# qingyundou/WaveRNN

Measured on AMD Instinct MI355X. Metric: audio samples/sec/GPU (22.05 kHz MoL, rnn_dims=512) + real-time factor at batch=1, higher is better.
Workload: dtype f32

## Files before the change

wavernn_amd/csrc/capi_loops.cpp:

```cpp
#include "host_ctx.h"

using namespace wrnn;
using namespace wrnn::host;

namespace {

struct DbgBuf {
    unsigned *p = nullptr;
    DbgBuf() = default;
    DbgBuf(const DbgBuf &) = delete;
    DbgBuf &operator=(const DbgBuf &) = delete;
    ~DbgBuf() {
        if (p) (void)hipFree(p);
    }
    unsigned *release() {
        unsigned *q = p;
        p = nullptr;
        return q;
    }
};

int dump_stamps(wrnn_t *h, DbgBuf &dbg, size_t n, const int (&hdr)[3], hipStream_t st) {
    std::vector<unsigned> host(n);
    HIP_TRY(h, hipStreamSynchronize(st));
// ... 190 lines not shown
            g1.B = group_rows(Bl, 1);
            g1.b0 = b0 + Bg;
        }
        HIP_TRY(h, launch_dm(a, grouped ? &g1 : nullptr, dm_lds_bytes(*h, Bg, TB), st));
        b0 += Bl;
    }
    return WRNN_OK;
}

int generate_split(wrnn_t *h, const float *cond, int B, int L, const float *noise, uint64_t seed,
                   int64_t row_offset, float *out, hipStream_t st) {
    const wrnn_config &c = h->cfg;
    const int R = c.rnn_dims, A = c.aux_dims, G = h->sGg + h->sGf, N = G * kSplitTerms;
    if (int rc = blas_on(h, st)) return rc;
    const double budget = terms_budget_floats();
    const int Lc_max = (int)std::max(1.0, std::min((double)L, budget / (double)(N + h->KX) - 1.0));
    const char *rep_env = std::getenv("WRNN_REPLICAS");
    const int reps = std::max(1, std::min(32, rep_env ? std::atoi(rep_env) : 4));
    const long long vec_max = std::max<long long>({(long long)kTermsPerUnit * R, (long long)R, (long long)c.fc_dims,
                                                   (long long)(R / kSplitUnits) * kYLine,
                                                   (long long)h->sGf * kSplitLogitLine});
    const long long rep_stride = (((vec_max + kOverRead) * 8 + 65535) / 65536) * 65536 / 8;
    const size_t need_xg = (size_t)kSplitHops * reps * rep_stride;
    HIP_TRY(h, ensure(h->d_xg, h->xg_cap, need_xg));
    if (grow(h, h->d_X, h->X_cap, (size_t)(Lc_max + 1) * h->KX) || grow(h, h->d_T, h->T_cap, (size_t)(Lc_max + 1) * N) ||
        grow(h, h->d_state, h->state_cap, (size_t)G * split_state_w(R)))
        return WRNN_EHIP;
    const char *dbg_env = std::getenv("WRNN_DEBUG_STAMPS");
    const int dbg_steps = dbg_env ? std::min(L, std::atoi(dbg_env)) : 0;
    DbgBuf dbg;
    if (dbg_steps > 0) {
        HIP_TRY(h, hipMalloc(&dbg.p, (size_t)G * dbg_steps * kStamps * 4));
        HIP_TRY(h, hipMemsetAsync(dbg.p, 0, (size_t)G * dbg_steps * kStamps * 4, st));
    }
    const float one = 1.0f, zero = 0.0f;
    for (int b0 = 0; b0 < B; ++b0) {
        HIP_TRY(h, hipMemsetAsync(h->d_xg, 0, need_xg * 8, st));
        for (int t0 = 0; t0 < L; t0 += Lc_max) {
            const int Lc = std::min(Lc_max, L - t0);
            const int rows = std::min(Lc + 1, L - t0);
            HIP_TRY(h, launch_ci_gemm(cond, h->CD, B, b0, 1, t0, rows, h->d_IW, 1 + c.feat_dims + A, h->d_Ib, R,
                                      c.feat_dims + A, h->d_X, h->KX, st));
            HIP_TRY(h, launch_pack_terms_input(cond, h->CD, B, b0, 1, t0, rows, c.feat_dims, A, R, h->KX, h->d_X, st));
            if (rocblas_sgemm(h->blas, rocblas_operation_transpose, rocblas_operation_none, N, rows, h->KX, &one,
                              h->d_sWt, h->KX, h->d_X, h->KX, &zero, h->d_T, N) != rocblas_status_success)
                return fail(h, WRNN_EHIP, "rocblas_sgemm (conditioning terms) failed");
            SplitArgs a{};
            a.gslab = h->d_sgslab;
            a.fslab = h->d_sfslab;
            a.terms = h->d_T;
            a.noise = noise;
            a.out = out;
            a.state = h->d_state;
            a.xg = h->d_xg;
            a.ctl = h->d_ctl;
            a.seed = seed;
            a.row0 = row_offset + b0;
            a.timeout_ticks = h->timeout_ticks;
            a.rep_stride = rep_stride;
            a.L = L;
            a.t0 = t0;
            a.Lc = Lc;
            a.Bt = B;
            a.b0 = b0;
            a.Gg = h->sGg;
            a.Gf = h->sGf;
            a.reps = reps;
            a.gs = h->sgs;
            a.fs = h->sfs;
            a.dbg = (b0 == 0 && t0 == 0) ? dbg.p : nullptr;
            a.dbg_steps = std::min(dbg_steps, Lc);
            HIP_TRY(h, launch_split(a, split_lds_bytes(*h), st));
        }
    }
    if (dbg.p) return dump_stamps(h, dbg, (size_t)G * dbg_steps * kStamps, {G, dbg_steps, kStamps}, st);
    return WRNN_OK;
}

template <typename Args, typename Slab>
int generate_xcd_rows(wrnn_t *h, const float *cond, const FrameSrc *fs, int B, int L, const float *noise,
                      uint64_t seed, int64_t row_offset, float *out, hipStream_t st, int n_terms, int state_w,
                      const Slab &slab, hipError_t (*launch)(const Args &, hipStream_t)) {
    const int N = kXcdWgs * n_terms;
    if (int rc = blas_on(h, st)) return rc;
    if (fs) {
        const float one = 1.0f, zero = 0.0f;
        const int rc = frame_terms(h, *fs, N, h->KXc, 0, st, [&](const float *X, int m, float *C) -> int {
            if (rocblas_sgemm(h->blas, rocblas_operation_transpose, rocblas_operation_none, N, m, h->KXc, &one,
                              h->d_xWt, h->KXc, X, h->KXc, &zero, C, N) != rocblas_status_success)
                return fail(h, WRNN_EHIP, "rocblas_sgemm (frame terms) failed");
            return WRNN_OK;
        });
        if (rc) return rc;
    }
    const double budget = terms_budget_floats();
    const size_t xg_words = (size_t)kXcds * kXXcdStride;
    if (!h->d_members) HIP_TRY(h, hipMalloc(&h->d_members, kXcds * sizeof(int)));
    if (!h->d_xgx) HIP_TRY(h, hipMalloc(&h->d_xgx, xg_words * 8));
    const char *dbg_env = std::getenv("WRNN_DEBUG_STAMPS");
    const int dbg_steps = dbg_env ? std::min(L, std::atoi(dbg_env)) : 0;
    DbgBuf dbg;
    int dbg_G = 0;
    const float one = 1.0f, zero = 0.0f;
    for (int b0 = 0; b0 < B; b0 += kXcds) {
        const int nb = std::min(kXcds, B - b0);
        const int Lc_max = (int)std::max(1.0, std::min((double)L, budget / ((double)nb * (N + h->KXc)) - 1.0));
        if (grow(h, h->d_X, h->X_cap, (size_t)(Lc_max + 1) * nb * h->KXc) ||
            grow(h, h->d_T, h->T_cap, (size_t)(Lc_max + 1) * nb * N) ||
            grow(h, h->d_xstate, h->xstate_cap, (size_t)nb * kXcdWgs * state_w))
            return WRNN_EHIP;
        if (dbg_steps > 0 && !dbg.p) {
            dbg_G = nb * kXcdWgs;
            HIP_TRY(h, hipMalloc(&dbg.p, (size_t)dbg_G * dbg_steps * kStamps * 4));
            HIP_TRY(h, hipMemsetAsync(dbg.p, 0, (size_t)dbg_G * dbg_steps * kStamps * 4, st));
        }
        HIP_TRY(h, hipMemsetAsync(h->d_xgx, 0, (size_t)nb * kXXcdStride * 8, st));
        for (int t0 = 0; t0 < L; t0 += Lc_max) {
            const int Lc = std::min(Lc_max, L - t0);
            const int rows = std::min(Lc + 1, L - t0);
            if (fs) {
                HIP_TRY(h, launch_terms_interp(h->d_FT, h->d_AT, fs->coef, h->d_T, N, fs->U, fs->NF, fs->NF + fs->nJ - 1,
                                               fs->hop, fs->nJ, fs->nf, fs->stride, fs->rb + b0, nb, t0, rows, st));
            } else {
                HIP_TRY(h, launch_pack_cond_input(cond, h->CD, B, b0, nb, t0, rows, h->KXc, h->d_X, st));
                if (rocblas_sgemm(h->blas, rocblas_operation_transpose, rocblas_operation_none, N, rows * nb, h->KXc,
                                  &one, h->d_xWt, h->KXc, h->d_X, h->KXc, &zero, h->d_T, N) != rocblas_status_success)
                    return fail(h, WRNN_EHIP, "rocblas_sgemm (conditioning terms) failed");
            }
            HIP_TRY(h, hipMemsetAsync(h->d_members, 0, kXcds * sizeof(int), st));
            Args a{};
            a.slab = h->d_xslab;
            a.terms = h->d_T;
            a.noise = noise;
            a.out = out;
            a.state = h->d_xstate;
            a.xg = h->d_xgx;
            a.members = h->d_members;
            a.ctl = h->d_ctl;
            a.seed = seed;
            a.row0 = row_offset + b0;
            a.timeout_ticks = h->timeout_ticks;
            a.L = L;
            a.t0 = t0;
            a.Lc = Lc;
            a.Bt = B;
            a.b0 = b0;
            a.nb = nb;
            a.s = slab;
            a.dbg = (b0 == 0 && t0 == 0) ? dbg.p : nullptr;
            a.dbg_steps = std::min(dbg_steps, Lc);
            HIP_TRY(h, launch(a, st));
        }
    }
    if (dbg.p) return dump_stamps(h, dbg, (size_t)dbg_G * dbg_steps * kStamps, {dbg_G, dbg_steps, kStamps}, st);
    return WRNN_OK;
}

int generate_xcd(wrnn_t *h, const float *cond, const FrameSrc *fs, int B, int L, const float *noise, uint64_t seed,
                 int64_t row_offset, float *out, hipStream_t st) {
    return generate_xcd_rows<XcdArgs>(h, cond, fs, B, L, noise, seed, row_offset, out, st, kXTerms, kXStateW, h->xs,
                                      launch_xcd);
}

int generate_xcds(wrnn_t *h, const float *cond, const FrameSrc *fs, int B, int L, const float *noise, uint64_t seed,
                  int64_t row_offset, float *out, hipStream_t st) {
    return generate_xcd_rows<XcdsArgs>(h, cond, fs, B, L, noise, seed, row_offset, out, st, kSTerms, kSStateW, h->xss,
                                       launch_xcds);
}

int generate_xcdm(wrnn_t *h, const float *cond, const FrameSrc *fs, int B, int L, const float *noise, uint64_t seed,
                  int64_t row_offset, float *out, int32_t *labels, hipStream_t st) {
    const int N = kXcdWgs * kMRing;
    const bool raw = h->cfg.mode == WRNN_MODE_RAW;
    const int NK = raw ? kMRawNC : 11;
    if (int rc = blas_on(h, st)) return rc;
    const double budget = terms_budget_floats();
    const size_t xg_words = (size_t)kXcds * kMXcdStride;
    if (!h->d_members) HIP_TRY(h, hipMalloc(&h->d_members, kXcds * sizeof(int)));
    if (!h->d_xmxg) HIP_TRY(h, hipMalloc(&h->d_xmxg, xg_words * 8));
    if (!h->d_xmstate) HIP_TRY(h, hipMalloc(&h->d_xmstate, (size_t)kXcds * kXcdWgs * kMStateW * sizeof(float)));
    const int rows_max = kXcds * 4 * h->xcdm_nq;
    const float one = 1.0f, zero = 0.0f;
    XcdmGemm gemms[3];
    xcdm_terms_gemms(*h, gemms);
    auto terms_gemm = [&](const float *X, int m, float *C) -> int {
        for (const XcdmGemm &g : gemms) {
            const rocblas_status rs =
                rocblas_sgemm(h->blas, rocblas_operation_transpose, rocblas_operation_none, g.rows, m, g.k, &one,
                              h->d_xmWt + (size_t)g.row0 * h->KXc + g.col0, h->KXc, X + g.col0, h->KXc, &zero,
                              C + g.row0, N);
            if (rs != rocblas_status_success) return fail(h, WRNN_EHIP, "rocblas_sgemm (conditioning terms) failed");
        }
        return WRNN_OK;
    };
    if (fs) {
        if (int rc = frame_terms(h, *fs, N, h->KXc, h->cfg.feat_dims + h->cfg.aux_dims, st, terms_gemm)) return rc;
    }
    const char *dbg_env = std::getenv("WRNN_DEBUG_STAMPS");
    const int dbg_steps = (!raw && dbg_env && std::atoi(dbg_env) > 0 && L >= kMDbgSkip + kMDbgSteps) ? kMDbgSteps : 0;
    const size_t dbg_n = (size_t)kXcds * kXcdWgs * kMWaves * dbg_steps * kMStamps;
    DbgBuf dbg;
    if (dbg_steps > 0) {
        HIP_TRY(h, hipMalloc(&dbg.p, dbg_n * 4));
        HIP_TRY(h, hipMemsetAsync(dbg.p, 0, dbg_n * 4, st));
    }
    for (int b0 = 0; b0 < B; b0 += rows_max) {
        const int nb = std::min(rows_max, B - b0);
        const int nq = (((nb + kXcds - 1) / kXcds) + 3) / 4;
        const int Lc_max = (int)std::max(1.0, std::min((double)L, budget / ((double)nb * (N + h->KXc + (noise ? 0 : NK)))));
        if (grow(h, h->d_X, h->X_cap, (size_t)Lc_max * nb * h->KXc) || grow(h, h->d_T, h->T_cap, (size_t)Lc_max * nb * N) ||
            (!noise && grow(h, h->d_xmnoise, h->xmnoise_cap, (size_t)Lc_max * nb * NK)))
// ... 488 lines not shown
```

wavernn_amd/csrc/fatchord_xcd.h:

```cpp
#pragma once
#include <hip/hip_runtime_api.h>
#include <stdint.h>

namespace wrnn {

constexpr int kXcds = 8;
constexpr int kXcdWgs = 32;
constexpr int kXWaves = 8;
constexpr int kXThreads = 64 * kXWaves;
constexpr int kXUnits = 16;
constexpr int kXFcRows = 16;
constexpr int kXWaveFc1 = 1, kXWaveFc2 = 3;
constexpr int kXH2RegRows = 30;
constexpr int kXH2LdsRows = 18;
static_assert(kXH2RegRows == 2 * (4 * 3 + 3 * 1), "W_hh2 VGPR passes: 3 on each fc wave, 1 on waves 5..7");
static_assert(kXH2RegRows + kXH2LdsRows == 48, "every W_hh2 row of the workgroup has one holder");
constexpr int kXRing = 4;
constexpr int kXNoise = 16;

enum XTerm { XT_P1 = 0, XT_P2 = 48, XT_CI = 96, XT_V1 = 112, XT_V2 = 128, kXTerms = 160 };

enum XHop { XH_Y = 0, XH_F1 = 1, XH_F2 = 2, XH_H2 = 3, XH_S0 = 4, XH_S1 = 5, kXHops = 6 };
constexpr int kXF2Line = 32;
constexpr long long kXHopStride = 4096;
constexpr long long kXXcdStride = kXHops * kXHopStride + 512;

struct XcdSlab {
    int wih2;
    int w1;
    int w2;
    int whh2;
    int whh1;
    int w3;
    int q1a;
    int cst;
    int total;
};

enum XCst { XC_Q2 = 0, XC_BIH1 = 48, XC_BHH1 = 96, XC_BIH2 = 144, XC_BHH2 = 192, XC_WI0 = 240, XC_B3 = 256, kXCst = 288 };

constexpr int kXStateW = 512 + 2048 + 48 + 16 + 16;

struct XcdArgs {
    const float *slab;
    const float *terms;
    const float *noise;
    float *out;
    float *state;
    unsigned long long *xg;
    int *members;
    int *ctl;
    unsigned long long seed;
    long long row0;
    long long timeout_ticks;
    int L, t0, Lc, Bt, b0, nb;
    XcdSlab s;
    unsigned *dbg;
    int dbg_steps;
    int windowed, nz_hor, out_ld, out_t0;
};

struct XcdRow {
    const float *terms;
    const float *noise;
    float *out;
    float *state;
    unsigned long long *xg;
    unsigned long long seed;
    long long row;
    long long terms_ld;
    int noise_ld;
    int out_t0;
    int t0, Lc, L, nz_hor;
};

struct XcdGroupArgs {
    XcdArgs a;
    XcdRow row[kXcds];
};

struct XcdPiece {
    XcdRow r;
    const float *ft;
    const float *at;
    int frames, nt;
    int blk0, pad_;
};

struct XcdListArgs {
    XcdArgs a;
    const XcdPiece *pieces;
    int first[kXcds + 1];
};

struct XcdLds {
    int whh1, whh2, h1, h2, sg, w3, f2x, ring, nz, gh2, cst, xs, misc, total;
};

__host__ __device__ constexpr XcdLds xcd_lds_layout() {
    XcdLds l{};
    int o = 0;
    l.h1 = o;    o += 512;
    l.h2 = o;    o += 512;
    l.sg = o;    o += 4 * 512;
    l.w3 = o;    o += kXFcRows * 32;
    l.f2x = o;   o += 64;
    l.ring = o;  o += kXRing * kXTerms;
    l.nz = o;    o += kXRing * kXNoise;
    l.gh2 = o;   o += 48;
    l.cst = o;   o += kXCst;
    l.xs = o;    o += 4;
    l.misc = o;  o += 8;
    l.whh1 = o;  o += 48 * 512;
    l.whh2 = o;  o += kXH2LdsRows * 512;
    l.total = o;
    return l;
}
static_assert(xcd_lds_layout().total * 4 <= 160 * 1024, "the XCD kernel's LDS image fits a CU's 160 KB");

hipError_t launch_xcd(const XcdArgs &a, hipStream_t st);
hipError_t launch_xcd_group(const XcdGroupArgs &g, hipStream_t st);
hipError_t launch_xcd_list(const XcdListArgs &g, hipStream_t st);
hipError_t prepare_xcd_kernel(int max_lds_bytes);
hipError_t xcd_occupancy(int *blocks_per_cu);

}
```

wavernn_amd/csrc/fatchord_xcd.hip:

```cpp
#include <hip/hip_runtime.h>
#include <stdint.h>

#include <type_traits>

#include "fatchord_loop.h"
#include "fatchord_xcd.h"
#include "wrnn_device.h"
#include "xcd_device.h"

namespace wrnn {

#ifndef WRNN_XCD_SKIP_SG
#define WRNN_XCD_SKIP_SG 0
#endif
#ifndef WRNN_XCD_SKIP_H2
#define WRNN_XCD_SKIP_H2 0
#endif
#ifndef WRNN_XCD_SKIP_RECUR
#define WRNN_XCD_SKIP_RECUR 0
#endif
#ifndef WRNN_XCD_PRIO
#define WRNN_XCD_PRIO 0
#endif

#ifndef WRNN_XCD_SQ3_WAVE
#define WRNN_XCD_SQ3_WAVE 4
#endif
#ifndef WRNN_XCD_STAMP_W13
#define WRNN_XCD_STAMP_W13 5
#endif
#define XSTAMPW(kk, w)                                                                                        \
    do {                                                                                                      \
        if (kDbg && a.dbg && wave == (w) && lane == 0 && t - t0 < a.dbg_steps &&                            \
            (!WRNN_XCD_BAR_STAMPS || ((kk) != 3 && ((kk) < 9 || (kk) > 14))))                                 \
            a.dbg[((size_t)mem * a.dbg_steps + (t - t0)) * kStamps + (kk)] = (unsigned)__builtin_amdgcn_s_memrealtime(); \
    } while (0)
#define XSTAMP(kk) XSTAMPW(kk, 0)
#define XSTAMP_BAR()                                                                                          \
    do {                                                                                                      \
        if (WRNN_XCD_BAR_STAMPS && kDbg && a.dbg && wave > 0 && lane == 0 && t - t0 < a.dbg_steps)          \
            a.dbg[((size_t)mem * a.dbg_steps + (t - t0)) * kStamps + (wave == 7 ? 3 : 8 + wave)] =          \
                (unsigned)__builtin_amdgcn_s_memrealtime();                                                   \
    } while (0)

#define XCD_PIECE_BEGIN()                                                                                     \
    do {                                                                                                      \
        {                                                                                                     \
            for (int t = t0; t < t0 + 3; ++t) {                                                               \
                if (t <= t_terms)                                                                             \
                    for (int i = tid; i < kXTerms; i += kXThreads) RING(t)[i] = TERMS(t)[i];                  \
                if (wave == 1 && lane < 11 && t < nz_hor) NZ(t)[lane] = noise_term(t);                        \
            }                                                                                                 \
        }                                                                                                     \
        resume = t0 > 0;                                                                                      \
        if constexpr (kGrp) st = rw.state + (size_t)c * kXStateW;                                             \
        else st = a.state + ((size_t)k * kXcdWgs + c) * kXStateW;                                             \
        h1v = resume ? st[tid] : 0.0f;                                                                        \
        h2own = resume ? st[512 + 2048 + 48 + ui] : 0.0f;                                                     \
        asm volatile("" : "+v"(h1v), "+v"(h2own));                                                            \
        if (resume) {                                                                                         \
            for (int i = tid; i < 4 * R; i += kXThreads) sg[i] = st[512 + i];                                 \
            if (tid < 48) gh2s[tid] = st[512 + 2048 + tid];                                                   \
            if (tid == 0) xs[(t0 + 1) & 1] = st[512 + 2048 + 48 + 16];                                        \
        } else {                                                                                              \
            if (tid < 48) gh2s[tid] = 0.0f;                                                                   \
            if (tid == 0) xs[1] = 0.0f;                                                                       \
        }                                                                                                     \
        __syncthreads();                                                                                      \
        if (!resume) {                                                                                        \
            if (gh1w) {                                                                                       \
                const float z5[5] = {0.0f, 0.0f, 0.0f, 0.0f, 0.0f};                                           \
                publish_terms(0, z5);                                                                         \
            }                                                                                                 \
            if (wave == 1 || wave == 2 || wave == 5 || wave == WRNN_XCD_SQ3_WAVE) {                           \
                asm volatile("s_waitcnt vmcnt(0)" ::: "memory");                                              \
                gather_terms(0);                                                                              \
            }                                                                                                 \
        }                                                                                                     \
        __syncthreads();                                                                                      \
        if (*abort_flag) return;                                                                              \
        x = xs[(t0 + 1) & 1];                                                                                 \
        s4 = lds4(sg + 4 * tid);                                                                              \
    } while (0)

#define XCD_PIECE_END()                                                                                       \
    do {                                                                                                      \
        __syncthreads();                                                                                      \
        st[tid] = h1v;                                                                                        \
        for (int i = tid; i < 4 * R; i += kXThreads) st[512 + i] = sg[i];                                     \
        if (tid < 48) st[512 + 2048 + tid] = gh2s[tid];                                                       \
        if (g2w && (li & ~2) == 0) st[512 + 2048 + 48 + ui] = h2own;                                          \
        if (tid == 0) st[512 + 2048 + 48 + 16] = xs[(t_end - 1) & 1];                                         \
    } while (0)

__device__ __forceinline__ const XcdArgs &launch_args(const XcdArgs &ka) { return ka; }
__device__ __forceinline__ const XcdArgs &launch_args(const XcdGroupArgs &ka) { return ka.a; }
__device__ __forceinline__ const XcdArgs &launch_args(const XcdListArgs &ka) { return ka.a; }

template <bool kDbg, bool kWin, bool kGrp = false, bool kLst = false>
__global__ __launch_bounds__(kXThreads, 2) void fatchord_xcd_kernel(
    std::conditional_t<kLst, XcdListArgs, std::conditional_t<kGrp, XcdGroupArgs, XcdArgs>> ka) {
    static_assert(!kGrp || (kWin && !kDbg), "grouped launches are windowed and carry no stamps");
    static_assert(!kLst || kGrp, "a list launch is a grouped one whose rows come from the piece queue");
    const XcdArgs &a = launch_args(ka);
    extern __shared__ __attribute__((aligned(16))) float smem[];
    constexpr int R = 512, TW = kXcdWgs * kXTerms;
    const XcdLds ll = xcd_lds_layout();
    const int tid = threadIdx.x, lane = tid & 63, li = lane & 31, eng = lane >> 5;
    const int wave = WRNN_XCD_UNIFORM_WAVE ? __builtin_amdgcn_readfirstlane(tid >> 6) : tid >> 6;
    float *whh1 = smem + ll.whh1, *whh2l = smem + ll.whh2, *f2x = smem + ll.f2x, *h1s = smem + ll.h1, *h2s = smem + ll.h2, *sg = smem + ll.sg, *w3s = smem + ll.w3;
    float *ring = smem + ll.ring, *nzr = smem + ll.nz, *gh2s = smem + ll.gh2, *cst = smem + ll.cst, *xs = smem + ll.xs;
    int *misc = reinterpret_cast<int *>(smem + ll.misc);
    int *abort_flag = misc, *h2ready = misc + 2, *ypub = misc + 3, *ygot = misc + 4, *f1got = misc + 5;

    if (tid == 0) {
        const int k = (int)xcc_id();
        int c = kXcdWgs;
        if constexpr (kLst) {
            const bool in = k < a.nb && ka.first[k + 1] > ka.first[k];
            if (in) c = atomicAdd(&a.members[k], 1);
            misc[1] = (in && c < kXcdWgs) ? k * kXcdWgs + c : -1;
        } else if constexpr (kGrp) {
            const bool in = k < a.nb && ka.row[k].Lc > 0;
            if (in) c = atomicAdd(&a.members[k], 1);
            misc[1] = (in && c < kXcdWgs) ? k * kXcdWgs + c : -1;
        } else {
            if (k < a.nb) c = atomicAdd(&a.members[k], 1);
            misc[1] = (k < a.nb && c < kXcdWgs) ? k * kXcdWgs + c : -1;
        }
        misc[0] = 0;
        for (int i = 2; i < 8; ++i) misc[i] = 0;
    }
    if (tid < 64) f2x[tid] = 0.0f;
    __syncthreads();
// ... 11 lines not shown
        t0 = rw.t0;
        Lc = rw.Lc;
        L = rw.L;
    } else if constexpr (kGrp) {
        rw = ka.row[k];
        t0 = rw.t0;
        Lc = rw.Lc;
        L = rw.L;
    } else {
        t0 = a.t0;
        Lc = a.Lc;
        L = a.L;
    }
    int t_end = t0 + Lc;
    int t_terms = min(t_end, L - 1);
    int nz_hor;
    if constexpr (kGrp) nz_hor = rw.nz_hor;
    else nz_hor = kWin ? a.nz_hor : L;
    unsigned long long *xg;
    if constexpr (kGrp) xg = rw.xg;
    else xg = a.xg + (size_t)k * kXXcdStride;
    auto XG = [&](int hop) { return xg + (size_t)hop * kXHopStride; };
    __amdgpu_buffer_rsrc_t xgr = __builtin_amdgcn_make_buffer_rsrc(xg, 0, 0x7fffffff, 0x00020000);
    auto XGI = [&](int hop) { return hop * (int)kXHopStride; };
    auto RING = [&](int t) { return ring + (t & (kXRing - 1)) * kXTerms; };
    auto NZ = [&](int t) { return nzr + (t & (kXRing - 1)) * kXNoise; };
    auto TERMS = [&](int t) {
        if constexpr (kGrp) return rw.terms + (size_t)(t - t0) * (size_t)rw.terms_ld + (size_t)c * kXTerms;
        else return a.terms + ((size_t)(t - t0) * a.nb + k) * TW + (size_t)c * kXTerms;
    };
    const float *S = a.slab + (size_t)c * a.s.total;
    unsigned long long prow, seed;
    if constexpr (kGrp) {
        prow = (unsigned long long)rw.row;
        seed = rw.seed;
    } else {
        prow = (unsigned long long)(a.row0 + k);
        seed = a.seed;
    }

    f4v W[28];
    auto ldrow = [&](const float *row, int m) { return *reinterpret_cast<const f4v *>(row + 4 * (li + 32 * m)); };
    const bool fcw = wave >= kXWaveFc1 && wave < kXWaveFc2 + 2;
    const bool g2w = !fcw;
    const int g2 = g2w && wave != 0 ? wave - 4 : 0;
    if (fcw) {
        const int hf = (wave - kXWaveFc1) & 1;
        const float *Wf = S + (wave < kXWaveFc2 ? a.s.w1 : a.s.w2) + hf * 8 * R;
#pragma unroll
        for (int p = 0; p < 4; ++p)
#pragma unroll
            for (int kk = 0; kk < 4; ++kk) {
                const f2v ra = *reinterpret_cast<const f2v *>(Wf + 2 * p * R + 2 * (lane + 64 * kk));
                const f2v rb = *reinterpret_cast<const f2v *>(Wf + (2 * p + 1) * R + 2 * (lane + 64 * kk));
                W[4 * p + kk] = f4v{ra.x, rb.x, ra.y, rb.y};
            }
#pragma unroll
        for (int p = 0; p < 3; ++p)
#pragma unroll
            for (int m = 0; m < 4; ++m) W[16 + 4 * p + m] = ldrow(S + a.s.whh2 + (2 * (3 * (wave - 1) + p) + eng) * R, m);
    } else {
        auto g2row = [&](int j, int q) { return S + a.s.wih2 + ((2 * g2 + j) * 6 + 2 * q + eng) * R; };
#pragma unroll
        for (int p = 0; p < 3; ++p) {
            const float *ra = g2row(p == 1 ? 1 : 0, p == 2 ? 2 : 0), *rb = g2row(p == 0 ? 0 : 1, p == 2 ? 2 : 1);
#pragma unroll
            for (int m = 0; m < 4; ++m) {
                const f4v wa = ldrow(ra, m), wb = ldrow(rb, m);
                W[8 * p + 2 * m] = f4v{wa.x, wb.x, wa.y, wb.y};
                W[8 * p + 2 * m + 1] = f4v{wa.z, wb.z, wa.w, wb.w};
            }
        }
#pragma unroll
        for (int m = 0; m < 4; ++m)
            W[24 + m] = wave != 0 ? ldrow(S + a.s.whh2 + (2 * (7 + wave) + eng) * R, m) : f4v{0.0f, 0.0f, 0.0f, 0.0f};
    }
    auto W4 = [&](int i) -> const f4v(&)[4] { return *reinterpret_cast<const f4v(*)[4]>(&W[i]); };
    auto W4x8 = [&](int i) -> const f4v(&)[8] { return *reinterpret_cast<const f4v(*)[8]>(&W[i]); };
    auto W4x16 = [&]() -> const f4v(&)[16] { return *reinterpret_cast<const f4v(*)[16]>(&W[0]); };
    const float q1r = S[a.s.q1a + tid], q1z = S[a.s.q1a + R + tid], q1n = S[a.s.q1a + 2 * R + tid];
    const int ui = 4 * g2 + (li & 2) + eng, gq = li & 1;
    const bool gh1w = wave == 0 || wave == 3 || wave == 4 || wave == 5 || wave == 7;
    const int gh0 = wave == 0 ? 0 : wave == 7 ? 40 : 10 * (wave - 2);
    auto noise_term = [&](int t) -> float {
        float uu;
        if constexpr (kGrp) {
            if (rw.noise) uu = rw.noise[(size_t)t * (size_t)rw.noise_ld + lane];
            else uu = philox_noise(seed, prow, (uint32_t)t, (uint32_t)lane, 1);
        } else {
            if (a.noise) uu = a.noise[((size_t)t * a.Bt + b) * 11 + lane];
            else uu = philox_noise(seed, prow, (uint32_t)t, (uint32_t)lane, 1);
        }
        return mol_noise_term(uu, lane);
    };
    auto publish_term = [&](int t, int rr, float gh) {
        const int u = rr / 3, q = rr - 3 * u;
        const float p1 = RING(t)[XT_P1 + rr], bh = cst[XC_BHH1 + rr], bi = cst[XC_BIH1 + rr];
        const int g = XGI(XH_S0 + (t & 1)) + (c * kXUnits + u) * 4;
        const uint32_t tag = (uint32_t)t + 1u;
        if (q < 2) {
            xpub_b(xgr, g + q, tag, (gh + bh) + (p1 + bi));
        } else {
            xpub_b(xgr, g + 3, tag, gh + bh);
            xpub_b(xgr, g + 2, tag, p1 + bi);
        }
    };
    auto publish_terms = [&](int t, const float (&gh)[5]) {
        const int rr = gh0 + 2 * li + eng;
        if (li < 5 && rr < 48) {
            const float v = li == 0 ? gh[0] : li == 1 ? gh[1] : li == 2 ? gh[2] : li == 3 ? gh[3] : gh[4];
            publish_term(t, rr, v);
        }
    };
    auto gh1_dots = [&](float (&gh)[5]) {
        f4v hx[4];
        e32x(h1s, li, hx);
#pragma unroll
        for (int p = 0; p < 5; ++p) {
            f4v w4[4];
            e32x(whh1 + min(gh0 + 2 * p + eng, 47) * R, li, w4);
            gh[p] = e32dot(w4, hx);
        }
    };
    auto set_flag = [&](int *f, uint32_t tag) {
        if (lane == 0) __hip_atomic_store(f, (int)tag, __ATOMIC_RELAXED, __HIP_MEMORY_SCOPE_WORKGROUP);
    };
    auto wait_flag = [&](int *f, uint32_t tag) {
        while (__hip_atomic_load(f, __ATOMIC_RELAXED, __HIP_MEMORY_SCOPE_WORKGROUP) != (int)tag)
            __builtin_amdgcn_s_sleep(1);
        asm volatile("" ::: "memory");
    };
    auto gh2_store = [&](int rb, int np, const float (&gh)[5]) {
        const int rr = rb + 2 * li + eng;
        if (li < np) gh2s[rr] = li == 0 ? gh[0] : li == 1 ? gh[1] : li == 2 ? gh[2] : li == 3 ? gh[3] : gh[4];
    };
    auto gh2_lds = [&](int p0, int np, const f4v (&hx)[4]) {
        float gh[5] = {0.0f, 0.0f, 0.0f, 0.0f, 0.0f};
#pragma unroll
        for (int p = 0; p < 2; ++p)
            if (p < np) {
                f4v w4[4];
                e32x(whh2l + (2 * (p0 + p) + eng - kXH2RegRows) * R, li, w4);
                gh[p] = e32dot(w4, hx);
            }
        gh2_store(2 * p0, np, gh);
    };
    auto gather_terms = [&](int t) {
        const int qq = wave == 1 ? 0 : wave == 2 ? 1 : wave == 5 ? 2 : 3;
        xgather16<4>(XG(XH_S0 + (t & 1)) + qq * 512, (uint32_t)t + 1u, a.ctl, a.timeout_ticks, t, XH_S0 + (t & 1),
                     abort_flag, lane, [&](int i, float v0, float v1) {
                         *reinterpret_cast<f2v *>(sg + qq * 512 + i) = f2v{v0, v1};
                     });
    };

    auto pub4 = [&](int hop, float v, uint32_t tagv) {
        const auto s = __builtin_amdgcn_permlane32_swap(__float_as_uint(v), __float_as_uint(v), false, false);
        if ((lane & ~2) == 0)
            __builtin_amdgcn_raw_buffer_store_b128(u4v{__float_as_uint(v), tagv, s[1], tagv}, xgr,
                                                   (XGI(hop) + c * kXUnits + 4 * g2 + lane) * 8, 0, 0);
    };
    {
        const f4v *src = reinterpret_cast<const f4v *>(S + a.s.whh1);
        f4v *dst = reinterpret_cast<f4v *>(whh1);
        for (int i = tid; i < 48 * R / 4; i += kXThreads) dst[i] = src[i];
        src = reinterpret_cast<const f4v *>(S + a.s.whh2 + kXH2RegRows * R);
        dst = reinterpret_cast<f4v *>(whh2l);
        for (int i = tid; i < kXH2LdsRows * R / 4; i += kXThreads) dst[i] = src[i];
        for (int i = tid; i < kXFcRows * 32; i += kXThreads) w3s[i] = S[a.s.w3 + i];
        for (int i = tid; i < kXCst; i += kXThreads) cst[i] = S[a.s.cst + i];
    }
    bool resume;
    float *st;
    float h1v, h2own;
    float x;
    f4v s4;
    XCD_PIECE_BEGIN();

    if (WRNN_XCD_PRIO && wave == 0) __builtin_amdgcn_s_setprio(WRNN_XCD_PRIO);
    for (int t = t0; t < t_end; ++t) {
        const uint32_t tag = (uint32_t)t + 1u;
        const bool more = t + 1 < L;
        const float *tr = RING(t);
        XSTAMP(0);
        if (kDbg && a.dbg && wave == 0 && lane == 0 && t - t0 < a.dbg_steps)
            a.dbg[((size_t)mem * a.dbg_steps + (t - t0)) * kStamps + 15] = (unsigned)__builtin_amdgcn_s_memtime();
        float q2v[2], p2v[2], bi2[2], ghv[2];
#pragma unroll
        for (int q = 0; q < 2; ++q) {
            const int gi = ui * 3 + (q == 0 ? gq : 2);
            q2v[q] = cst[XC_Q2 + gi];
            p2v[q] = tr[XT_P2 + gi];
            bi2[q] = cst[XC_BIH2 + gi];
            ghv[q] = gh2s[gi] + cst[XC_BHH2 + gi];
        }
        const float wi0v = cst[XC_WI0 + ui], civ = tr[XT_CI + ui];
        {
            const float r = sigmoid_(fmaf(x, q1r, s4.x));
            const float z = sigmoid_(fmaf(x, q1z, s4.y));
            const float n = tanh_(fmaf(x, q1n, s4.z) + s4.w * r);
            h1v = (h1v - n) * z + n;
            h1s[tid] = h1v;
        }
        float p2q[2];
#pragma unroll
        for (int q = 0; q < 2; ++q) p2q[q] = fmaf(x, q2v[q], p2v[q]) + bi2[q];
        const float xi = fmaf(wi0v, x, civ);
        bar();
        XSTAMP(1);
        if (g2w) {
            f4v hx[4];
            e32x(h1s, li, hx);
            float yb = xi + h1s[c * kXUnits + ui];
            uint32_t tagv = tag;
            asm volatile("" : "+v"(yb), "+v"(tagv));
            const f2v ga = e32part2(W4x8(0), hx), gb = e32part2(W4x8(8), hx);
            const float g_s = e32rs4(ga.x, ga.y, gb.x, gb.y, lane);
            const float s = sigmoid_(ghv[0] + (g_s + p2q[0]));
            const f2v gn = e32part2(W4x8(16), hx);
            const float g_n = e32rs2(gn.x, gn.y, lane);
            const float z = WRNN_DPP(s, 0xF5);
            const float n = tanh_((g_n + p2q[1]) + ghv[1] * s);
            const float hn = (h2own - n) * z + n;
            h2own = hn;
            pub4(XH_Y, yb + hn, tagv);
            if (wave == 0) set_flag(ypub, tag);
        }
        XSTAMP(2);
        auto pub_h2 = [&]() { pub4(XH_H2, h2own, tag); };
        const int jq = lane & 1, rho = jq + 2 * (lane >> 4);
        if (wave == 0) {
            if (more && !WRNN_XCD_SKIP_RECUR) {
                float gh[5];
                gh1_dots(gh);
                wait_flag(ygot, tag);
                publish_terms(t + 1, gh);
                pub_h2();
            }
            const int jp = lane & 15, pg = lane >> 4;
            const float ua = NZ(t)[jp < 5 ? 2 * jp : 0], ub = NZ(t)[jp < 5 ? 2 * jp + 1 : 0], u10 = NZ(t)[10];
            const float b3a = cst[XC_B3 + 2 * jp], b3b = cst[XC_B3 + 2 * jp + 1];
            asm volatile("s_waitcnt vmcnt(0)" ::: "memory");
            const __amdgpu_buffer_rsrc_t rf = hop_rsrc(XG(XH_F2));
            const int goff = pg * 8 * kXF2Line * 8 + jp * 16;
            const unsigned long long c0 = __builtin_amdgcn_s_memrealtime();
            unsigned spins = 0;
            u4v v[8];
            for (;;) {
#pragma unroll
                for (int m = 0; m < 8; ++m) v[m] = ld16_sc1(rf, goff + m * kXF2Line * 8);
                bool ok = true;
#pragma unroll
                for (int m = 0; m < 8; ++m) ok &= (v[m].y == tag) & (v[m].w == tag);
                if (__ballot(!ok) == 0) break;
                if ((++spins & 63u) == 0) {
                    const bool late = (long long)(__builtin_amdgcn_s_memrealtime() - c0) > a.timeout_ticks;
                    const bool other = __hip_atomic_load(&a.ctl[0], __ATOMIC_RELAXED, __HIP_MEMORY_SCOPE_AGENT) != 0;
                    if (late || other) {
                        if (late) record_abort(a.ctl, -4, t, XH_F2, blockIdx.x);
                        *abort_flag = 1;
#pragma unroll
                        for (int m = 0; m < 8; ++m) v[m] = u4v{0u, 0u, 0u, 0u};
                        break;
                    }
                }
            }
            float pa[8], pb[8];
#pragma unroll
            for (int m = 0; m < 8; ++m) {
                pa[m] = __uint_as_float(v[m].x);
                pb[m] = __uint_as_float(v[m].z);
            }
            XSTAMP(7);
#pragma unroll
            for (int n = 4; n >= 1; n /= 2)
#pragma unroll
                for (int m = 0; m < n; ++m) {
                    pa[m] += pa[m + n];
                    pb[m] += pb[m + n];
                }
            cross_rows_pair(pa[0], pb[0]);
            const float la = pa[0] + b3a, lb = pb[0] + b3b;
            x = mol_sample_pairs(la, lb, ua, ub, u10, jp);
            if (lane == 0) {
                xs[t & 1] = x;
                if constexpr (kGrp) {
                    if (c == 0) rw.out[t - rw.out_t0] = x;
                } else {
                    if (c == 0) a.out[kWin ? (size_t)b * a.out_ld + (t - a.out_t0) : (size_t)b * L + t] = x;
                }
            }
            XSTAMP(8);
        } else if (wave < kXWaveFc2) {
            const int hf = wave - kXWaveFc1, rg = 8 * hf + rho;
            const float v1 = tr[XT_V1 + rg];
            asm volatile("s_waitcnt vmcnt(0)" ::: "memory");
            u4v v[4];
            xpoll16<4>(XG(XH_Y), tag, a.ctl, a.timeout_ticks, t, XH_Y, abort_flag, lane, v);
            if (hf == 0) set_flag(ygot, tag);
            XSTAMPW(3, 1);
            float o[2];
            fc8_rows_rp(W4x16(), v, o);
            const float A = (jq == 0 ? o[0] : o[1]) + v1;
            if ((lane & 15) < 2) xpub_b(xgr, XGI(XH_F1) + c * kXFcRows + rg, tag, A > 0.0f ? A : 0.0f);
            XSTAMPW(4, 1);
            if (more && !WRNN_XCD_SKIP_RECUR) {
                wait_flag(f1got, tag);
                if (!WRNN_XCD_SKIP_SG) {
                    asm volatile("s_waitcnt vmcnt(0)" ::: "memory");
                    gather_terms(t + 1);
                }
                wait_flag(h2ready, tag);
                f4v hx[4];
                e32x(h2s, li, hx);
                const float gh[5] = {e32dot(W4(16), hx), e32dot(W4(20), hx), e32dot(W4(24), hx), 0.0f, 0.0f};
                gh2_store(6 * hf, 3, gh);
                gh2_lds(15 + 2 * hf, 2, hx);
                XSTAMPW(11, 1);
            }
        } else if (wave < kXWaveFc2 + 2) {
            const int hf = wave - kXWaveFc2;
            if (more && !WRNN_XCD_SKIP_RECUR) {
                wait_flag(ypub, tag);
                float gh[5];
                gh1_dots(gh);
                wait_flag(ygot, tag);
                publish_terms(t + 1, gh);
            }
            XSTAMPW(9, 3);
            float v2[2], w3c[8];
#pragma unroll
            for (int j = 0; j < 2; ++j) v2[j] = tr[XT_V2 + 8 * hf + j + 2 * (lane >> 4)];
#pragma unroll
            for (int r = 0; r < 8; ++r) w3c[r] = w3s[(8 * hf + r) * 32 + li];
            asm volatile("s_waitcnt vmcnt(0)" ::: "memory");
            u4v v[4];
            xpoll16<4>(XG(XH_F1), tag, a.ctl, a.timeout_ticks, t, XH_F1, abort_flag, lane, v);
            if (hf == 0) set_flag(f1got, tag);
            XSTAMPW(5, 3);
            float o[2];
            fc8_rows_rp(W4x16(), v, o);
            float p = 0.0f;
#pragma unroll
            for (int j = 0; j < 2; ++j) {
                const float f = o[j] + v2[j];
                const float f2 = f > 0.0f ? f : 0.0f;
#pragma unroll
                for (int g = 0; g < 4; ++g) p = fmaf(w3c[j + 2 * g], lane_bcast(f2, 16 * g), p);
            }
            unsigned long long *f2p = reinterpret_cast<unsigned long long *>(f2x);
            if (hf == 1) {
                if (lane < 32)
                    __hip_atomic_store(f2p + lane, ((unsigned long long)tag << 32) | __float_as_uint(p), __ATOMIC_RELAXED,
                                       __HIP_MEMORY_SCOPE_WORKGROUP);
            } else {
                unsigned spin = 0;
                unsigned long long pv = (unsigned long long)tag << 32;
                for (;;) {
                    if (lane < 32) pv = __hip_atomic_load(f2p + lane, __ATOMIC_RELAXED, __HIP_MEMORY_SCOPE_WORKGROUP);
                    if (__ballot((uint32_t)(pv >> 32) != tag) == 0) break;
                    if ((++spin & 255u) == 0 &&
                        __hip_atomic_load(abort_flag, __ATOMIC_RELAXED, __HIP_MEMORY_SCOPE_WORKGROUP))
                        break;
                }
                if (lane < kXF2Line)
                    xpub_b(xgr, XGI(XH_F2) + c * kXF2Line + lane, tag, p + __uint_as_float((uint32_t)pv));
                XSTAMPW(6, 3);
            }
            if ((WRNN_XCD_SQ3_WAVE == 3 || WRNN_XCD_SQ3_WAVE == 4) && wave == WRNN_XCD_SQ3_WAVE && more &&
                !WRNN_XCD_SKIP_RECUR && !WRNN_XCD_SKIP_SG) {
                asm volatile("s_waitcnt vmcnt(0)" ::: "memory");
                gather_terms(t + 1);
            }
            if (more && !WRNN_XCD_SKIP_RECUR) {
                wait_flag(h2ready, tag);
                f4v hx[4];
                e32x(h2s, li, hx);
                const float gh[5] = {e32dot(W4(16), hx), e32dot(W4(20), hx), e32dot(W4(24), hx), 0.0f, 0.0f};
                gh2_store(12 + 6 * hf, 3, gh);
                if (hf == 0) gh2_lds(22, 2, hx);
            }
        } else if (more) {
            if (WRNN_XCD_SKIP_RECUR) {
                if (wave == 7) {
                    wait_flag(f1got, tag);
                    if (t + 2 >= t0 + 3) {
                        if (t + 2 <= t_terms && lane < kXTerms / 4)
                            reinterpret_cast<f4v *>(RING(t + 2))[lane] = reinterpret_cast<const f4v *>(TERMS(t + 2))[lane];
                        if (t + 2 < nz_hor && lane < 11) NZ(t + 2)[lane] = noise_term(t + 2);
                    }
                }
                goto step_end;
            }
            if (wave != 6) {
                float gh[5];
                gh1_dots(gh);
                wait_flag(ygot, tag);
                publish_terms(t + 1, gh);
            } else {
                wait_flag(ygot, tag);
            }
            pub_h2();
            wait_flag(f1got, tag);
            if (wave == 6) {
                if (!WRNN_XCD_SKIP_H2) {
                    asm volatile("s_waitcnt vmcnt(0)" ::: "memory");
                    xgather16<4>(XG(XH_H2), tag, a.ctl, a.timeout_ticks, t, XH_H2, abort_flag, lane,
                                 [&](int i, float v0, float v1) { *reinterpret_cast<f2v *>(h2s + i) = f2v{v0, v1}; });
                }
                asm volatile("s_waitcnt lgkmcnt(0)" ::: "memory");
                set_flag(h2ready, tag);
                XSTAMPW(10, 6);
            }
            if (wave <= 6) {
                if (!WRNN_XCD_SKIP_SG && (wave == 5 || WRNN_XCD_SQ3_WAVE == 6)) {
                    asm volatile("s_waitcnt vmcnt(0)" ::: "memory");
                    gather_terms(t + 1);
                }
                XSTAMPW(14, 5);
            } else if (t + 2 >= t0 + 3) {
                if (t + 2 <= t_terms && lane < kXTerms / 4)
                    reinterpret_cast<f4v *>(RING(t + 2))[lane] = reinterpret_cast<const f4v *>(TERMS(t + 2))[lane];
                if (t + 2 < nz_hor && lane < 11) NZ(t + 2)[lane] = noise_term(t + 2);
                XSTAMPW(12, 7);
            }
            wait_flag(h2ready, tag);
            {
                f4v hx[4];
                e32x(h2s, li, hx);
                const float gh[5] = {e32dot(W4(24), hx), 0.0f, 0.0f, 0.0f, 0.0f};
                gh2_store(2 * (7 + wave), 1, gh);
                if (wave != 7) gh2_lds(wave == 5 ? 19 : 20, wave == 5 ? 1 : 2, hx);
                XSTAMPW(13, WRNN_XCD_STAMP_W13);
            }
        }
    step_end:
        XSTAMP_BAR();
        bar();
        const int ab = *abort_flag;
        const float xn = xs[t & 1];
        s4 = lds4(sg + 4 * tid);
        if (ab) return;
        if (wave != 0) x = xn;
        if constexpr (kLst) {
            if (t + 1 == t_end) {
                XCD_PIECE_END();
                if (++pi >= pend) return;
                rw = list_piece<XcdRow>(ka.pieces, pi);
                t0 = rw.t0;
                Lc = rw.Lc;
                L = rw.L;
                t_end = t0 + Lc;
                t_terms = min(t_end, L - 1);
                nz_hor = rw.nz_hor;
                xg = rw.xg;
                xgr = __builtin_amdgcn_make_buffer_rsrc(xg, 0, 0x7fffffff, 0x00020000);
                prow = (unsigned long long)rw.row;
                seed = rw.seed;
                __syncthreads();
                if (tid < 64) f2x[tid] = 0.0f;
                if (tid >= 64 && tid < 70) misc[tid - 62] = 0;
                XCD_PIECE_BEGIN();
                t = t0 - 1;
            }
        }
    }
    if constexpr (!kLst) XCD_PIECE_END();
}

#define WRNN_K_XCD fatchord_xcd_kernel<false, false>
#define WRNN_K_XCD_DBG fatchord_xcd_kernel<true, false>
#define WRNN_K_XCD_WIN fatchord_xcd_kernel<false, true>
#define WRNN_K_XCD_GRP fatchord_xcd_kernel<false, true, true>
#define WRNN_K_XCD_LST fatchord_xcd_kernel<false, true, true, true>

hipError_t launch_xcd(const XcdArgs &a, hipStream_t st) {
    XcdArgs args = a;
    void *params[] = {&args};
    const void *kf = a.windowed ? (const void *)WRNN_K_XCD_WIN : a.dbg ? (const void *)WRNN_K_XCD_DBG : (const void *)WRNN_K_XCD;
    return hipLaunchKernel(kf, dim3(kXcds * kXcdWgs), dim3(kXThreads), params, xcd_lds_layout().total * sizeof(float), st);
}

hipError_t launch_xcd_group(const XcdGroupArgs &g, hipStream_t st) {
    XcdGroupArgs args = g;
    void *params[] = {&args};
    return hipLaunchKernel((const void *)WRNN_K_XCD_GRP, dim3(kXcds * kXcdWgs), dim3(kXThreads), params,
                           xcd_lds_layout().total * sizeof(float), st);
}

hipError_t launch_xcd_list(const XcdListArgs &g, hipStream_t st) {
    XcdListArgs args = g;
    void *params[] = {&args};
    return hipLaunchKernel((const void *)WRNN_K_XCD_LST, dim3(kXcds * kXcdWgs), dim3(kXThreads), params,
                           xcd_lds_layout().total * sizeof(float), st);
}

hipError_t prepare_xcd_kernel(int max_lds_bytes) {
    for (const void *kf : {(const void *)WRNN_K_XCD, (const void *)WRNN_K_XCD_DBG, (const void *)WRNN_K_XCD_WIN,
                           (const void *)WRNN_K_XCD_GRP, (const void *)WRNN_K_XCD_LST}) {
        hipError_t e = hipFuncSetAttribute(kf, hipFuncAttributeMaxDynamicSharedMemorySize, max_lds_bytes);
        if (e != hipSuccess) return e;
    }
    return hipSuccess;
}

hipError_t xcd_occupancy(int *blocks_per_cu) {
    int best = 1 << 30;
    for (const void *kf : {(const void *)WRNN_K_XCD, (const void *)WRNN_K_XCD_DBG, (const void *)WRNN_K_XCD_WIN,
                           (const void *)WRNN_K_XCD_GRP, (const void *)WRNN_K_XCD_LST}) {
        int n = 0;
        hipError_t e = hipOccupancyMaxActiveBlocksPerMultiprocessor(&n, kf, kXThreads, xcd_lds_layout().total * sizeof(float));
        if (e != hipSuccess) return e;
        best = n < best ? n : best;
    }
    *blocks_per_cu = best;
    return hipSuccess;
}

}
```

wavernn_amd/csrc/host_ctx.h:

```cpp
#pragma once
#include <hip/hip_runtime.h>
#include <rocblas/rocblas.h>

#include <algorithm>
#include <climits>
#include <cmath>
#include <cstdio>
#include <cstdlib>
#include <cstring>
#include <map>
#include <memory>
#include <string>
#include <vector>

#include "../../include/wavernn_amd.h"
#include "condition.h"
#include "deepmind_rows.h"
#include "deepmind_xcd.h"
#include "fatchord_loop.h"
#include "fatchord_rows.h"
#include "fatchord_split.h"
#include "fatchord_xcd.h"
#include "fatchord_xcdm.h"
#include "fatchord_xcds.h"
#include "frame_terms.h"

namespace wrnn {
namespace host {

template <typename T>
hipError_t ensure(T *&p, size_t &cap, size_t n) {
    if (n <= cap) return hipSuccess;
    if (p) {
        hipError_t e = hipFree(p);
        if (e != hipSuccess) return e;
    }
    p = nullptr;
    cap = 0;
    hipError_t e = hipMalloc(&p, n * sizeof(T));
    if (e == hipSuccess) cap = n;
    return e;
}

template <typename Rec>
struct StagedTable {
    Rec *d = nullptr, *h = nullptr;
    size_t d_cap = 0, h_cap = 0;
    hipEvent_t ev = nullptr;

    hipError_t reserve(size_t n) {
        hipError_t e = ev ? hipSuccess : hipEventCreateWithFlags(&ev, hipEventDisableTiming);
        if (e == hipSuccess) e = hipEventSynchronize(ev);
        if (e == hipSuccess) e = ensure(d, d_cap, n);
        if (e != hipSuccess || n <= h_cap) return e;
        if (h && (e = hipHostFree(h)) != hipSuccess) return e;
        h = nullptr;
        h_cap = 0;
        e = hipHostMalloc((void **)&h, 2 * n * sizeof(Rec), hipHostMallocDefault);
        if (e == hipSuccess) h_cap = 2 * n;
        return e;
    }
    hipError_t upload(size_t n, hipStream_t st) {
        hipError_t e = hipMemcpyAsync(d, h, n * sizeof(Rec), hipMemcpyHostToDevice, st);
        return e == hipSuccess ? hipEventRecord(ev, st) : e;
    }
    void release() {
        if (d) (void)hipFree(d);
        if (h) (void)hipHostFree(h);
        if (ev) (void)hipEventDestroy(ev);
        d = h = nullptr;
        d_cap = h_cap = 0;
        ev = nullptr;
    }
};

}
}

struct RowsPart {
    wrnn::RowsSlab rs{};
    int rU = 0, rG = 0, rUF = 0, rUC = 0, NT = 0;
    bool ok = false;
    float *d_slab = nullptr, *d_Wt = nullptr;
};

struct DmPart {
    wrnn::DmSlab ds{};
    int dmU = 0, dmUO = 0, dmUO2 = 0, G = 0;
    bool ok = false;
    float *d_slab = nullptr;
};

struct wrnn_ctx {
    wrnn_config cfg{};
    int device = 0;
// ... 218 lines not shown
```

Before: 323,800.

## Precompute sampler noise draws into terms padding and panel the conditioning GEMM

A new pre-pass kernel computes the per-step MoL noise terms (from supplied noise or Philox) and writes them into the unused tail of each workgroup's terms record. The recurrent XCD kernel then reads them from the terms ring instead of generating them on its critical path, except in windowed mode. The conditioning GEMM is split into fixed-width column panels, and the buffers are rounded up to whole panels. A flag wait on the f2 exchange is also added before the sampler reads, which adds synchronization that could cost time.

```diff
diff --git a/wavernn_amd/csrc/capi_loops.cpp b/wavernn_amd/csrc/capi_loops.cpp
--- a/wavernn_amd/csrc/capi_loops.cpp
+++ b/wavernn_amd/csrc/capi_loops.cpp
@@ -296,6 +296,8 @@
                       uint64_t seed, int64_t row_offset, float *out, hipStream_t st, int n_terms, int state_w,
                       const Slab &slab, hipError_t (*launch)(const Args &, hipStream_t)) {
     const int N = kXcdWgs * n_terms;
+    constexpr bool kPanels = std::is_same_v<Args, XcdArgs>;
+    constexpr int kTermsPanel = 8192;
     if (int rc = blas_on(h, st)) return rc;
     if (fs) {
         const float one = 1.0f, zero = 0.0f;
@@ -319,8 +321,9 @@
     for (int b0 = 0; b0 < B; b0 += kXcds) {
         const int nb = std::min(kXcds, B - b0);
         const int Lc_max = (int)std::max(1.0, std::min((double)L, budget / ((double)nb * (N + h->KXc)) - 1.0));
-        if (grow(h, h->d_X, h->X_cap, (size_t)(Lc_max + 1) * nb * h->KXc) ||
-            grow(h, h->d_T, h->T_cap, (size_t)(Lc_max + 1) * nb * N) ||
+        const size_t cols_max = (size_t)(Lc_max + 1) * nb;
+        const size_t cols_cap = kPanels ? (cols_max + kTermsPanel - 1) / kTermsPanel * kTermsPanel : cols_max;
+        if (grow(h, h->d_X, h->X_cap, cols_cap * h->KXc) || grow(h, h->d_T, h->T_cap, cols_cap * N) ||
             grow(h, h->d_xstate, h->xstate_cap, (size_t)nb * kXcdWgs * state_w))
             return WRNN_EHIP;
         if (dbg_steps > 0 && !dbg.p) {
@@ -337,10 +340,15 @@
                                                fs->hop, fs->nJ, fs->nf, fs->stride, fs->rb + b0, nb, t0, rows, st));
             } else {
                 HIP_TRY(h, launch_pack_cond_input(cond, h->CD, B, b0, nb, t0, rows, h->KXc, h->d_X, st));
-                if (rocblas_sgemm(h->blas, rocblas_operation_transpose, rocblas_operation_none, N, rows * nb, h->KXc,
-                                  &one, h->d_xWt, h->KXc, h->d_X, h->KXc, &zero, h->d_T, N) != rocblas_status_success)
-                    return fail(h, WRNN_EHIP, "rocblas_sgemm (conditioning terms) failed");
+                const int cols = rows * nb, step = kPanels ? kTermsPanel : cols;
+                for (int c0 = 0; c0 < cols; c0 += step)
+                    if (rocblas_sgemm(h->blas, rocblas_operation_transpose, rocblas_operation_none, N, step, h->KXc,
+                                      &one, h->d_xWt, h->KXc, h->d_X + (size_t)c0 * h->KXc, h->KXc, &zero,
+                                      h->d_T + (size_t)c0 * N, N) != rocblas_status_success)
+                        return fail(h, WRNN_EHIP, "rocblas_sgemm (conditioning terms) failed");
             }
+            if constexpr (std::is_same_v<Args, XcdArgs>)
+                HIP_TRY(h, launch_xcd_draws(h->d_T, noise, seed, row_offset + b0, nb, B, b0, t0, rows, st));
             HIP_TRY(h, hipMemsetAsync(h->d_members, 0, kXcds * sizeof(int), st));
             Args a{};
             a.slab = h->d_xslab;
diff --git a/wavernn_amd/csrc/fatchord_xcd.h b/wavernn_amd/csrc/fatchord_xcd.h
--- a/wavernn_amd/csrc/fatchord_xcd.h
+++ b/wavernn_amd/csrc/fatchord_xcd.h
@@ -18,7 +18,8 @@
 constexpr int kXRing = 4;
 constexpr int kXNoise = 16;
 
-enum XTerm { XT_P1 = 0, XT_P2 = 48, XT_CI = 96, XT_V1 = 112, XT_V2 = 128, kXTerms = 160 };
+enum XTerm { XT_P1 = 0, XT_P2 = 48, XT_CI = 96, XT_V1 = 112, XT_V2 = 128, XT_NZ = 144, kXTerms = 160 };
+static_assert(XT_NZ + kXNoise == kXTerms, "the sampler record fills the terms record's padding");
 
 enum XHop { XH_Y = 0, XH_F1 = 1, XH_F2 = 2, XH_H2 = 3, XH_S0 = 4, XH_S1 = 5, kXHops = 6 };
 constexpr int kXF2Line = 32;
@@ -119,6 +120,8 @@
 static_assert(xcd_lds_layout().total * 4 <= 160 * 1024, "the XCD kernel's LDS image fits a CU's 160 KB");
 
 hipError_t launch_xcd(const XcdArgs &a, hipStream_t st);
+hipError_t launch_xcd_draws(float *terms, const float *noise, unsigned long long seed, long long row0, int nb, int Bt,
+                            int b0, int t0, int n, hipStream_t st);
 hipError_t launch_xcd_group(const XcdGroupArgs &g, hipStream_t st);
 hipError_t launch_xcd_list(const XcdListArgs &g, hipStream_t st);
 hipError_t prepare_xcd_kernel(int max_lds_bytes);
diff --git a/wavernn_amd/csrc/fatchord_xcd.hip b/wavernn_amd/csrc/fatchord_xcd.hip
--- a/wavernn_amd/csrc/fatchord_xcd.hip
+++ b/wavernn_amd/csrc/fatchord_xcd.hip
@@ -25,6 +25,9 @@
 
 #ifndef WRNN_XCD_SQ3_WAVE
 #define WRNN_XCD_SQ3_WAVE 4
+#endif
+#ifndef WRNN_XCD_F2_GATE
+#define WRNN_XCD_F2_GATE 1
 #endif
 #ifndef WRNN_XCD_STAMP_W13
 #define WRNN_XCD_STAMP_W13 5
@@ -49,7 +52,8 @@
             for (int t = t0; t < t0 + 3; ++t) {                                                               \
                 if (t <= t_terms)                                                                             \
                     for (int i = tid; i < kXTerms; i += kXThreads) RING(t)[i] = TERMS(t)[i];                  \
-                if (wave == 1 && lane < 11 && t < nz_hor) NZ(t)[lane] = noise_term(t);                        \
+                if constexpr (kWin)                                                                           \
+                    if (wave == 1 && lane < 11 && t < nz_hor) NZ(t)[lane] = noise_term(t);                    \
             }                                                                                                 \
         }                                                                                                     \
         resume = t0 > 0;                                                                                      \
@@ -227,7 +231,7 @@
     const int ui = 4 * g2 + (li & 2) + eng, gq = li & 1;
     const bool gh1w = wave == 0 || wave == 3 || wave == 4 || wave == 5 || wave == 7;
     const int gh0 = wave == 0 ? 0 : wave == 7 ? 40 : 10 * (wave - 2);
-    auto noise_term = [&](int t) -> float {
+    [[maybe_unused]] auto noise_term = [&](int t) -> float {
         float uu;
         if constexpr (kGrp) {
             if (rw.noise) uu = rw.noise[(size_t)t * (size_t)rw.noise_ld + lane];
@@ -382,9 +386,11 @@
                 pub_h2();
             }
             const int jp = lane & 15, pg = lane >> 4;
-            const float ua = NZ(t)[jp < 5 ? 2 * jp : 0], ub = NZ(t)[jp < 5 ? 2 * jp + 1 : 0], u10 = NZ(t)[10];
+            const float *nzt = kWin ? NZ(t) : tr + XT_NZ;
+            const float ua = nzt[jp < 5 ? 2 * jp : 0], ub = nzt[jp < 5 ? 2 * jp + 1 : 0], u10 = nzt[10];
             const float b3a = cst[XC_B3 + 2 * jp], b3b = cst[XC_B3 + 2 * jp + 1];
             asm volatile("s_waitcnt vmcnt(0)" ::: "memory");
+            if (WRNN_XCD_F2_GATE) wait_flag(reinterpret_cast<int *>(f2x) + 1, tag);
             const __amdgpu_buffer_rsrc_t rf = hop_rsrc(XG(XH_F2));
             const int goff = pg * 8 * kXF2Line * 8 + jp * 16;
             const unsigned long long c0 = __builtin_amdgcn_s_memrealtime();
@@ -531,7 +537,8 @@
                     if (t + 2 >= t0 + 3) {
                         if (t + 2 <= t_terms && lane < kXTerms / 4)
                             reinterpret_cast<f4v *>(RING(t + 2))[lane] = reinterpret_cast<const f4v *>(TERMS(t + 2))[lane];
-                        if (t + 2 < nz_hor && lane < 11) NZ(t + 2)[lane] = noise_term(t + 2);
+                        if constexpr (kWin)
+                            if (t + 2 < nz_hor && lane < 11) NZ(t + 2)[lane] = noise_term(t + 2);
                     }
                 }
                 goto step_end;
@@ -565,7 +572,8 @@
             } else if (t + 2 >= t0 + 3) {
                 if (t + 2 <= t_terms && lane < kXTerms / 4)
                     reinterpret_cast<f4v *>(RING(t + 2))[lane] = reinterpret_cast<const f4v *>(TERMS(t + 2))[lane];
-                if (t + 2 < nz_hor && lane < 11) NZ(t + 2)[lane] = noise_term(t + 2);
+                if constexpr (kWin)
+                    if (t + 2 < nz_hor && lane < 11) NZ(t + 2)[lane] = noise_term(t + 2);
                 XSTAMPW(12, 7);
             }
             wait_flag(h2ready, tag);
@@ -618,6 +626,29 @@
 #define WRNN_K_XCD_GRP fatchord_xcd_kernel<false, true, true>
 #define WRNN_K_XCD_LST fatchord_xcd_kernel<false, true, true, true>
 
+__global__ void xcd_draws_kernel(float *terms, const float *noise, unsigned long long seed, long long row0, int nb, int Bt,
+                                 int b0, int t0, int n) {
+    const long long i = (long long)blockIdx.x * blockDim.x + threadIdx.x;
+    if (i >= (long long)n * nb * kXNoise) return;
+    const int kk = (int)(i % kXNoise), lr = (int)((i / kXNoise) % nb), t = t0 + (int)(i / ((long long)kXNoise * nb));
+    float v = 0.0f;
+    if (kk < 11) {
+        const float uu = noise ? noise[((size_t)t * Bt + b0 + lr) * 11 + kk]
+                               : philox_noise(seed, (unsigned long long)(row0 + lr), (uint32_t)t, (uint32_t)kk, 1);
+        v = mol_noise_term(uu, kk);
+    }
+    float *rec = terms + (size_t)(i / kXNoise) * (kXcdWgs * kXTerms) + XT_NZ + kk;
+    for (int c = 0; c < kXcdWgs; ++c) rec[(size_t)c * kXTerms] = v;
+}
+
+hipError_t launch_xcd_draws(float *terms, const float *noise, unsigned long long seed, long long row0, int nb, int Bt,
+                            int b0, int t0, int n, hipStream_t st) {
+    const long long m = (long long)n * nb * kXNoise;
+    hipLaunchKernelGGL(xcd_draws_kernel, dim3((unsigned)((m + 255) / 256)), dim3(256), 0, st, terms, noise, seed, row0,
+                       nb, Bt, b0, t0, n);
+    return hipGetLastError();
+}
+
 hipError_t launch_xcd(const XcdArgs &a, hipStream_t st) {
     XcdArgs args = a;
     void *params[] = {&args};
diff --git a/wavernn_amd/csrc/host_ctx.h b/wavernn_amd/csrc/host_ctx.h
--- a/wavernn_amd/csrc/host_ctx.h
+++ b/wavernn_amd/csrc/host_ctx.h
@@ -11,6 +11,7 @@
 #include <map>
 #include <memory>
 #include <string>
+#include <type_traits>
 #include <vector>
 
 #include "../../include/wavernn_amd.h"
```

Result: faster. 328,300, median of 6 (+1.4%).
